# Coloquinte/sleekit

Measured on AMD Instinct MI355X. Metric: Mweights/sec quantized (GPTQ 3-bit, 4096x4096 layer), higher is better.
Workload: dtype f64

## Files before the change

### sleekit_amd/csrc/api.hip

```cpp
#include "mfma32.h"
#include "mfma64.h"

namespace slk {

__global__ __launch_bounds__(256) void k_probe_f64(double *sink, int iters) {
    double4_t c0 = {0, 0, 0, 0}, c1 = c0, c2 = c0, c3 = c0;
    const double a = 1.0 + threadIdx.x * 1e-3, b = 1.0 - threadIdx.x * 1e-3;
    for (int i = 0; i < iters; ++i) {
        c0 = __builtin_amdgcn_mfma_f64_16x16x4f64(a, b, c0, 0, 0, 0);
        c1 = __builtin_amdgcn_mfma_f64_16x16x4f64(b, a, c1, 0, 0, 0);
        c2 = __builtin_amdgcn_mfma_f64_16x16x4f64(a, a, c2, 0, 0, 0);
        c3 = __builtin_amdgcn_mfma_f64_16x16x4f64(b, b, c3, 0, 0, 0);
    }
    const double4_t s = c0 + c1 + c2 + c3;
    if (s[0] + s[1] + s[2] + s[3] == 12345.678) sink[0] = s[0];
}

template <int NACC>
__global__ __launch_bounds__(256) void k_probe_f64_n(double *sink, int iters) {
    double4_t c[NACC];
    double a[NACC], b[NACC];
#pragma unroll
    for (int i = 0; i < NACC; ++i) {
        c[i] = (double4_t){0, 0, 0, 0};
// ... 51 lines not shown
    } else if (mode == 6) {
        CHAIN(x0 = (double)(float)x0 * a;)
    } else if (mode == 7) {
        CHAIN(x0 = __longlong_as_double(((long long)__builtin_amdgcn_readlane((int)(__double_as_longlong(x0) >> 32), 5) << 32) | 7) * a;)
    } else {
        CHAIN(f = rintf(f * 1.0000001f) + 0.25f;)
    }
#undef CHAIN
    const unsigned long long t1 = __builtin_amdgcn_s_memtime(), r1 = __builtin_amdgcn_s_memrealtime();
    if (threadIdx.x == 0) {
        out[0] = (double)(t1 - t0);
        out[1] = (double)(r1 - r0);
        out[2] = x0 + x1 + x2 + x3 + x4 + x5 + x6 + x7 + f;
    }
}

}

using namespace slk;

extern "C" {

int slk_probe_chain(double *out, int iters, int mode, slk_stream_t stream) {
    SLK_REQUIRE(out && iters > 0, "bad arguments");
    hipStream_t s = as_stream(stream);
    SLK_RUN("probe_chain", 0, 0, s, k_probe_chain<<<1, 64, 0, s>>>(out, iters, mode));
    return SLK_OK;
}

size_t slk_workspace_bytes(int R, int n) {
    if (R < 0 || n <= 0) return 0;
    const size_t ld = (size_t)slk_factor_ld(n);
    const size_t rn = (size_t)(R > 0 ? R : 1) * (size_t)n;
    size_t factor = 2 * ld * ld * sizeof(double) + 2 * (ld / 64) * sizeof(int);
    size_t loop = 2 * rn * sizeof(float) + (size_t)n * sizeof(int) + 64 * sizeof(float) + 5 * 256;
    size_t search = rn * sizeof(float) + (size_t)(R + n) * sizeof(float) + (size_t)R * ((n + 127) / 128) * sizeof(float) + 4096;
    size_t error = 6 * (rn + 128 * (size_t)n) + 6 * (size_t)n * n + 4 * (size_t)R * ((n + 127) / 128) * sizeof(float) + 8192;
    size_t prep = 64 * sizeof(float) + (size_t)n * (sizeof(double) + 1);
    search += error;
    size_t m = factor;
    if (loop > m) m = loop;
    if (search > m) m = search;
    if (error > m) m = error;
    if (prep > m) m = prep;
    return m + (1u << 16);
}

size_t slk_workspace_bytes_batch(int batch, int rows_per_layer, int n) {
    if (batch < 1 || batch > 64 || rows_per_layer < 0 || n <= 0 || (long long)batch * rows_per_layer > 0x7fffffffLL) return 0;
    return slk_workspace_bytes(batch * rows_per_layer, n) + (size_t)(batch - 1) * 6 * (size_t)n * n +
           (size_t)batch * n * (sizeof(int) + sizeof(float)) + (size_t)(batch - 1) * 64 * sizeof(float) +
           4096;
}

int slk_probe_mfma_f64(double *sink, int blocks, int iters, slk_stream_t stream) {
    SLK_REQUIRE(sink && blocks > 0 && iters > 0, "bad arguments");
    hipStream_t s = as_stream(stream);
    SLK_RUN("probe_mfma_f64", 4.0 * 2048 * 4 * iters * blocks, 0, s, k_probe_f64<<<blocks, 256, 0, s>>>(sink, iters));
    return SLK_OK;
}

int slk_probe_mfma_f64_acc(double *sink, int blocks, int iters, int nacc, slk_stream_t stream) {
    SLK_REQUIRE(sink && blocks > 0 && iters > 0 && (nacc == 1 || nacc == 2 || nacc == 4 || nacc == 8 || nacc == 16), "bad arguments");
    hipStream_t s = as_stream(stream);
    if (nacc == 1)
        SLK_RUN("probe_mfma_f64", 1.0 * 2048 * 4 * iters * blocks, 0, s, k_probe_f64_n<1><<<blocks, 256, 0, s>>>(sink, iters));
    else if (nacc == 2)
        SLK_RUN("probe_mfma_f64", 2.0 * 2048 * 4 * iters * blocks, 0, s, k_probe_f64_n<2><<<blocks, 256, 0, s>>>(sink, iters));
    else if (nacc == 4)
        SLK_RUN("probe_mfma_f64", 4.0 * 2048 * 4 * iters * blocks, 0, s, k_probe_f64_n<4><<<blocks, 256, 0, s>>>(sink, iters));
    else if (nacc == 8)
        SLK_RUN("probe_mfma_f64", 8.0 * 2048 * 4 * iters * blocks, 0, s, k_probe_f64_n<8><<<blocks, 256, 0, s>>>(sink, iters));
    else
        SLK_RUN("probe_mfma_f64", 16.0 * 2048 * 4 * iters * blocks, 0, s, k_probe_f64_n<16><<<blocks, 256, 0, s>>>(sink, iters));
    return SLK_OK;
}

int slk_probe_mfma_f32(float *sink, int blocks, int iters, slk_stream_t stream) {
    SLK_REQUIRE(sink && blocks > 0 && iters > 0, "bad arguments");
    hipStream_t s = as_stream(stream);
    SLK_RUN("probe_mfma_f32", 4.0 * 4096 * 4 * iters * blocks, 0, s, k_probe_f32<<<blocks, 256, 0, s>>>(sink, iters));
    return SLK_OK;
}

}

#include <atomic>
#include <map>
#include <mutex>
#include <string>
#include <vector>
#include <strings.h>

namespace slk {
namespace {
const char *const kOptNames[OPT_COUNT] = {
    "NO_FAST_LEAF", "NO_DEFER", "NO_WINDOW2", "WIN_DBG", "NO_REGULAR_SEARCH", "NO_FAST_SEARCH_DIV",
    "NO_ERROR_SPLITK", "ERROR_CB", "NO_SYM_ERROR", "NO_BF16_ERROR", "NO_BF16_DMA", "NO_BF16_HESSIAN",
    "ERROR_F32_BELOW", "NO_BF16_ASYM", "NO_SYM_AVERAGE", "NO_WAVE_SEARCH", "LOOKAHEAD", "WINDOW_ROWS", "PANEL_SPLIT", "ROWS_BELOW_WIDE",
    "NO_LOOP_ERROR", "CHAIN_CARRIES_BELOW",
};
std::atomic<int> g_opts[OPT_COUNT];
std::once_flag g_opts_once;
void opts_from_env() {
    for (int i = 0; i < OPT_COUNT; ++i) {
        const std::string name = std::string("SLK_") + kOptNames[i];
        const char *v = getenv(name.c_str());
        int val = 0;
        if (v) {
            val = atoi(v);
            if (val == 0 && v[0] != '0') val = 1;
        }
        g_opts[i].store(val, std::memory_order_relaxed);
    }
}
int opt_index(const char *name) {
    if (!name) return -1;
    if (strncasecmp(name, "SLK_", 4) == 0) name += 4;
    for (int i = 0; i < OPT_COUNT; ++i)
        if (strcasecmp(name, kOptNames[i]) == 0) return i;
    return -1;
}
std::mutex g_lds_mu;
std::map<std::pair<const void *, int>, size_t> g_lds_set;
}

int opt(Opt o) {
    std::call_once(g_opts_once, opts_from_env);
    return g_opts[o].load(std::memory_order_relaxed);
}

namespace {
std::mutex g_helper_mu;
// ... 206 lines not shown
```

### sleekit_amd/csrc/common.h

```cpp
#pragma once

#include <hip/hip_runtime.h>
#include <stddef.h>
#include <stdint.h>
#include <stdio.h>

#include <type_traits>

#include "../../include/sleekit_amd.h"

namespace slk {

void set_error(const char *fmt, ...);

#define SLK_REQUIRE(cond, ...)          \
    do {                                \
        if (!(cond)) {                  \
            slk::set_error(__VA_ARGS__); \
            return SLK_E_ARG;           \
        }                               \
    } while (0)

#define SLK_HIP(call)                                                                  \
    do {                                                                               \
// ... 23 lines not shown
        }                                                        \
        SLK_LAUNCH_CHECK();                                      \
    } while (0)

#define SLK_RUN_W(name, flops, bytes, wgs, stream, ...) \
    do {                                                \
        slk::prof_next_width((long)(wgs));              \
        SLK_RUN(name, flops, bytes, stream, __VA_ARGS__); \
    } while (0)

enum Opt {
    OPT_NO_FAST_LEAF,
    OPT_NO_DEFER,
    OPT_NO_WINDOW2,
    OPT_WIN_DBG,
    OPT_NO_REGULAR_SEARCH,
    OPT_NO_FAST_SEARCH_DIV,
    OPT_NO_ERROR_SPLITK,
    OPT_ERROR_CB,
    OPT_NO_SYM_ERROR,
    OPT_NO_BF16_ERROR,
    OPT_NO_BF16_DMA,
    OPT_NO_BF16_HESSIAN,
    OPT_ERROR_F32_BELOW,
    OPT_NO_BF16_ASYM,
    OPT_NO_SYM_AVERAGE,
    OPT_NO_WAVE_SEARCH,
    OPT_LOOKAHEAD,
    OPT_WINDOW_ROWS,
    OPT_PANEL_SPLIT,
    OPT_ROWS_BELOW_WIDE,
    OPT_NO_LOOP_ERROR,
    OPT_CHAIN_CARRIES_BELOW,
    OPT_COUNT
};
int opt(Opt o);

struct Helper {
    hipStream_t stream;
    hipStream_t stream2;
    hipEvent_t *events;
};
constexpr int HELPER_EVENTS = 512;
hipError_t helper_for(hipStream_t main, int need, Helper *out);

hipError_t lds_opt_in(const void *kernel, size_t bytes);
#define SLK_LDS_OPT_IN(kernel, bytes) SLK_HIP(slk::lds_opt_in(reinterpret_cast<const void *>(kernel), (bytes)))

struct PtrTable {
    const float *p[64];
};

constexpr int LOOP_LAYERS = 16;
struct LayerTable {
    const float *W[LOOP_LAYERS], *scale[LOOP_LAYERS];
    const long long *order[LOOP_LAYERS];
    const double *U[LOOP_LAYERS];
};
template <class T>
__device__ __forceinline__ const T *layer_base(const T *const (&column)[LOOP_LAYERS], int b, size_t stride) {
    return column[b % LOOP_LAYERS] + (size_t)(b - b % LOOP_LAYERS) * stride;
}

int row_errors_products(const float *W, const float *Q, const float *const *Hs, int batch, int rpl, int n, const int *sym_known,
                        float *row_err, float *G, void *workspace, size_t ws_bytes, slk_stream_t stream);

// ... 182 lines not shown
```

### sleekit_amd/csrc/factor.hip

```cpp
#include <stdlib.h>

#include "mfma64.h"

namespace slk {

constexpr int PANEL = 64;
constexpr int OUTER_SMALL = 256, OUTER_LARGE = 512;
constexpr int LOOKAHEAD_MIN_TILES = 24;

__device__ long long g_panel_cycles[16];

constexpr int TP = 66;

struct PanelSmem {
    double t[PANEL][TP];
    double x[PANEL][TP];
    double a21[PANEL][TP];
    double lb[PANEL][TP];
    double rdiag[PANEL];
    int early_count;
};

#ifndef NEWTON_STEPS
#define NEWTON_STEPS 2
#endif
__device__ __forceinline__ double rsqrt_newton(double d) {
    double y = __builtin_amdgcn_rsq(d);
#pragma unroll
    for (int it = 0; it < NEWTON_STEPS; ++it) {
        const double e = __builtin_fma(-(d * y), y, 1.0);
        y = __builtin_fma(0.5 * y, e, y);
    }
    return y;
}

__device__ __forceinline__ double4_t blk_load_d(const double *blk, int lane) {
    double4_t c;
#pragma unroll
    for (int r = 0; r < 4; ++r) c[r] = blk[((lane >> 4) + 4 * r) * TP + (lane & 15)];
    return c;
}
__device__ __forceinline__ void blk_store_d(double *blk, int lane, double4_t c) {
#pragma unroll
    for (int r = 0; r < 4; ++r) blk[((lane >> 4) + 4 * r) * TP + (lane & 15)] = c[r];
}
__device__ __forceinline__ double4_t blk_mma_abt(const double *a, const double *bt, double4_t acc, double sign, int lane) {
    const int o = (lane & 15) * TP + (lane >> 4);
#pragma unroll
    for (int g = 0; g < 4; ++g) acc = __builtin_amdgcn_mfma_f64_16x16x4f64(sign * a[o + 4 * g], bt[o + 4 * g], acc, 0, 0, 0);
    return acc;
}
__device__ __forceinline__ double4_t blk_mma_ab(const double *a, const double *b, double4_t acc, int lane) {
    const int oa = (lane & 15) * TP + (lane >> 4), ob = (lane >> 4) * TP + (lane & 15);
// ... 336 lines not shown
            for (int cb = 0; cb < 4; ++cb) {
                double4_t acc = {0.0, 0.0, 0.0, 0.0};
#pragma unroll
                for (int kq = 0; kq < 4; ++kq) acc = blk_mma_abt(&sm.lb[16 * wave][16 * kq], &sm.lk[16 * cb][16 * kq], acc, 1.0, lane);
                double *cp = &sm.a21[16 * wave][16 * cb];
                double4_t o = blk_load_d(cp, lane);
#pragma unroll
                for (int r = 0; r < 4; ++r) o[r] = o[r] - acc[r];
                blk_store_d(cp, lane, o);
            }
            asm volatile("s_waitcnt lgkmcnt(0)" ::: "memory");
        }
#pragma unroll
        for (int cb = 0; cb < 4; ++cb) {
            double4_t acc = {0.0, 0.0, 0.0, 0.0};
#pragma unroll
            for (int k = 0; k < 4; ++k)
                if (k <= cb) acc = blk_mma_abt(&sm.a21[16 * wave][16 * k], &sm.x[16 * cb][16 * k], acc, 1.0, lane);
#pragma unroll
            for (int r = 0; r < 4; ++r) A[(size_t)(r0 + 16 * wave + (lane >> 4) + 4 * r) * ld + k0 + 16 * cb + (lane & 15)] = acc[r];
        }
        if (rt + 1 < last) __syncthreads();
    }
}


constexpr int INFO_HANDOFF_TIMEOUT = 0x7fffffff;
constexpr bool slk_chain_addressable(int ld) { return (size_t)ld * (size_t)ld * sizeof(double) <= 0xffffffffull; }

typedef unsigned int u32x4_t __attribute__((ext_vector_type(4)));
typedef unsigned int u32x2_t __attribute__((ext_vector_type(2)));
constexpr int AUX_SC1 = 16;
constexpr int CHAIN_CARRY_CAP = 80;
constexpr bool CHAIN_CARRY_BY_RULE = true;

struct GBuf {
    __amdgpu_buffer_rsrc_t rs;
    __device__ __forceinline__ GBuf(const double *base, size_t bytes)
        : rs(__builtin_amdgcn_make_buffer_rsrc(const_cast<double *>(base), 0, (int)(bytes > 0xffffffffull ? 0xffffffffull : bytes), 0x00020000)) {}
    template <int AUX>
    __device__ __forceinline__ double2_t load2(unsigned elem) const {
        const u32x4_t v = __builtin_amdgcn_raw_buffer_load_b128(rs, elem * 8u, 0, AUX);
        return (double2_t){__hiloint2double((int)v[1], (int)v[0]), __hiloint2double((int)v[3], (int)v[2])};
    }
    template <int AUX>
    __device__ __forceinline__ void store2(unsigned elem, double2_t x) const {
        const u32x4_t v = {(unsigned)__double2loint(x[0]), (unsigned)__double2hiint(x[0]), (unsigned)__double2loint(x[1]), (unsigned)__double2hiint(x[1])};
        __builtin_amdgcn_raw_buffer_store_b128(v, rs, elem * 8u, 0, AUX);
    }
};

__device__ __forceinline__ int flag_peek(const int *p) { return __hip_atomic_load(p, __ATOMIC_RELAXED, __HIP_MEMORY_SCOPE_AGENT); }
__device__ __forceinline__ bool flag_wait(const int *p, int want) {
    bool ok = flag_peek(p) >= want;
    if (!ok) {
        const unsigned long long t0 = __builtin_amdgcn_s_memrealtime();
        for (;;) {
            __builtin_amdgcn_s_sleep(1);
            if (flag_peek(p) >= want) {
                ok = true;
                break;
            }
            if (__builtin_amdgcn_s_memrealtime() - t0 > 200000000ull) break;
        }
    }
    __builtin_amdgcn_fence(__ATOMIC_ACQUIRE, "wavefront");
    return ok;
}
__device__ __forceinline__ void flag_publish(int *p, int value) {
    asm volatile("s_waitcnt vmcnt(0)" ::: "memory");
    __syncthreads();
    if (threadIdx.x == 0) __hip_atomic_store(p, value, __ATOMIC_RELAXED, __HIP_MEMORY_SCOPE_AGENT);
}

struct TileRegs {
    double2_t v[8];
};
template <int AUX, int J0 = 0, int J1 = 8>
__device__ __forceinline__ void tile_fetch(TileRegs &r, const GBuf &g, unsigned elem0, int ld) {
    const int t = threadIdx.x;
#pragma unroll
    for (int j = J0; j < J1; ++j) r.v[j] = g.load2<AUX>(elem0 + (unsigned)(8 * j + (t >> 5)) * (unsigned)ld + 2u * (t & 31));
}
template <int J0 = 0, int J1 = 8>
__device__ __forceinline__ void tile_stash(double (*img)[TP], const TileRegs &r) {
    const int t = threadIdx.x;
#pragma unroll
    for (int j = J0; j < J1; ++j) *reinterpret_cast<double2_t *>(&img[8 * j + (t >> 5)][2 * (t & 31)]) = r.v[j];
}
template <int AUX, int J0 = 0, int J1 = 8>
__device__ __forceinline__ void tile_store_from_lds(const GBuf &g, unsigned elem0, int ld, const double (*img)[TP]) {
    const int t = threadIdx.x;
#pragma unroll
    for (int j = J0; j < J1; ++j)
        g.store2<AUX>(elem0 + (unsigned)(8 * j + (t >> 5)) * (unsigned)ld + 2u * (t & 31), *reinterpret_cast<const double2_t *>(&img[8 * j + (t >> 5)][2 * (t & 31)]));
}

template <class Early>
__device__ __forceinline__ int diag_tile_factor(PanelSmem &sm, int lane, int wave, Early rows_0_and_1_are_in) {
    auto diag_inverse = [&](int kb) {
        const int c0 = 16 * kb, c = lane & 15;
        double xv[16];
#pragma unroll
        for (int i = 0; i < 16; ++i) {
            double s = 0.0;
#pragma unroll
            for (int u = 0; u < i; ++u) s = __builtin_fma(sm.t[c0 + i][c0 + u], xv[u], s);
            xv[i] = ((c == i ? 1.0 : 0.0) - s) * sm.rdiag[c0 + i];
        }
        if (lane < 16) {
#pragma unroll
            for (int i = 0; i < 16; ++i) sm.x[c0 + i][c0 + c] = xv[i];
        }
    };
    auto block_owner = [](int rb, int cb) { return cb == 1 ? rb : (rb == 3 && cb == 2 ? 2 : 1); };
    auto block_update = [&](int rb, int cb, int kb) {
        double *c = &sm.t[16 * rb][16 * cb];
        blk_store_d(c, lane, blk_mma_abt(&sm.t[16 * rb][16 * kb], &sm.t[16 * cb][16 * kb], blk_load_d(c, lane), -1.0, lane));
    };
    auto x_inner = [&](int rb, int cb) {
        double4_t sacc = {0.0, 0.0, 0.0, 0.0};
#pragma unroll
        for (int k = 0; k < 4; ++k)
            if (k >= cb && k < rb) sacc = blk_mma_ab(&sm.t[16 * rb][16 * k], &sm.x[16 * k][16 * cb], sacc, lane);
        return sacc;
// ... 37 lines not shown
            own_writes();
            if (kb == 2) x_block(1, 0);
            if (kb == 3) {
                x_block(2, 1);
                x_block(2, 0);
            }
        } else {
#pragma unroll
            for (int rb = kb + 1; rb < 4; ++rb)
#pragma unroll
                for (int cb = kb + 1; cb <= rb; ++cb)
                    if (block_owner(rb, cb) == wave) block_update(rb, cb, kb - 1);
            if (kb == 3) rows_0_and_1_are_in(wave - 1);
        }
        __syncthreads();
        if (kb < 3) {
#pragma unroll
            for (int rb = kb + 1; rb < 4; ++rb)
                if (block_owner(rb, kb + 1) == wave) block_update(rb, kb + 1, kb);
            __syncthreads();
        }
    }
    double4_t row3 = {0.0, 0.0, 0.0, 0.0};
    if (wave == 3) diag_inverse(3);
    else row3 = x_inner(3, wave);
    __syncthreads();
    if (wave < 3) x_finish(3, wave, row3);
    __syncthreads();
    return first_bad;
}

enum ChainForm { CHAIN_ROWS, BELOW_ROWS, CHAIN_AND_BELOW };
template <int FORM>
__device__ __forceinline__ void chol_chain_walk(PanelSmem &sm, double *__restrict__ Aall, int ld, int K0, int nb, double *__restrict__ Xall,
                                                int *__restrict__ info, int *__restrict__ flags_all, int dbg) {
    const bool BELOW = FORM == BELOW_ROWS || (FORM == CHAIN_AND_BELOW && (int)blockIdx.x >= nb);
    constexpr bool WAITS = FORM != BELOW_ROWS;
    const int t = threadIdx.x, lane = t & 63, wave = t >> 6;
    const int r = FORM == BELOW_ROWS ? nb + (int)blockIdx.x : (int)blockIdx.x, nt = ld / PANEL, p0 = K0 / PANEL;
    const int rq = BELOW ? nb : r;
    const size_t mat = (size_t)ld * ld;
    double *A = Aall + (size_t)blockIdx.z * mat;
    const GBuf ga(A, mat * sizeof(double)), gx(Xall + (size_t)blockIdx.z * mat, mat * sizeof(double));
    info += blockIdx.z;
    int *xready = flags_all + (size_t)blockIdx.z * 2 * nt, *rowdone = xready + nt;
    const int row0 = K0 + PANEL * r;
    auto elem = [&](int tr, int tc) { return (unsigned)(K0 + PANEL * tr) * (unsigned)ld + (unsigned)(K0 + PANEL * tc); };
    bool alive = true;
    if (t == 0) sm.early_count = 0;
    const bool timing = !BELOW && dbg && r > 0 && blockIdx.z == 0 && wave == 0;
    long long tmark = 0;
    auto lap = [&](int slot) {
        if (timing) {
            const long long now = (long long)__builtin_readcyclecounter();
            if (lane == 0 && slot >= 0) atomicAdd(reinterpret_cast<unsigned long long *>(&g_panel_cycles[slot]), (unsigned long long)(now - tmark));
            tmark = now;
        }
    };

    double4_t tp[3];
    if (!BELOW) {
        int i = 0;
#pragma unroll
        for (int rb = 0; rb < 4; ++rb)
#pragma unroll
            for (int cb = 0; cb <= rb; ++cb, ++i)
                if ((i & 3) == wave) {
#pragma unroll
                    for (int j = 0; j < 4; ++j) {
                        const int rr = 16 * rb + (lane >> 4) + 4 * j, cc = 16 * cb + (lane & 15);
                        tp[i >> 2][j] = (r > 0 || cc <= rr) ? A[(size_t)(row0 + rr) * ld + row0 + cc] : 0.0;
                    }
                }
    }
    auto update_cn = [&](double4_t(&cn)[4]) {
#pragma unroll
        for (int cb = 0; cb < 4; ++cb) {
            double4_t acc = {0.0, 0.0, 0.0, 0.0};
#pragma unroll
            for (int kq = 0; kq < 4; ++kq) acc = blk_mma_abt(&sm.lb[16 * wave][16 * kq], &sm.t[16 * cb][16 * kq], acc, 1.0, lane);
#pragma unroll
            for (int j = 0; j < 4; ++j) cn[cb][j] = cn[cb][j] - acc[j];
        }
    };

    auto row_done = [&](int count) {
        if (BELOW) {
            asm volatile("s_waitcnt vmcnt(0)" ::: "memory");
            __syncthreads();
        } else {
            flag_publish(&rowdone[p0 + r], count);
        }
    };
    if (rq > 0) {
        TileRegs ra, rb_;
        double4_t cn[4];
        tile_fetch<0>(ra, ga, elem(r, 0), ld);
        tile_stash(sm.a21, ra);
        for (int q = 0; q < rq; ++q) {
            const bool more = q + 1 < rq;
            if (more) {
#pragma unroll
                for (int cb = 0; cb < 4; ++cb)
#pragma unroll
                    for (int j = 0; j < 4; ++j)
                        cn[cb][j] = A[(size_t)(row0 + 16 * wave + (lane >> 4) + 4 * j) * ld + K0 + PANEL * (q + 1) + 16 * cb + (lane & 15)];
                if (q > 0) {
                    if (WAITS) alive = alive && flag_wait(&rowdone[p0 + q + 1], 1);
                    tile_fetch<AUX_SC1>(ra, ga, elem(r, 0), ld);
                    tile_fetch<AUX_SC1>(rb_, ga, elem(q + 1, 0), ld);
                }
                for (int s = 0; s < q; ++s) {
                    __syncthreads();
                    tile_stash(sm.lb, ra);
                    tile_stash(sm.t, rb_);
                    __syncthreads();
                    if (s + 1 < q) {
                        if (WAITS && alive) alive = flag_wait(&rowdone[p0 + q + 1], s + 2);
                        tile_fetch<AUX_SC1>(ra, ga, elem(r, s + 1), ld);
                        tile_fetch<AUX_SC1>(rb_, ga, elem(q + 1, s + 1), ld);
                    }
                    update_cn(cn);
                }
            }
            const bool last = !BELOW && q + 1 == r;
            auto l_block = [&](int cb) {
                double4_t acc = {0.0, 0.0, 0.0, 0.0};
#pragma unroll
                for (int k = 0; k < 4; ++k)
                    if (k <= cb) acc = blk_mma_abt(&sm.a21[16 * wave][16 * k], &sm.x[16 * cb][16 * k], acc, 1.0, lane);
                blk_store_d(&sm.lb[16 * wave][16 * cb], lane, acc);
            };
            double4_t tacc[3];
            auto t_terms = [&](int kq0, int kq1) {
                int i = 0;
#pragma unroll
                for (int rb = 0; rb < 4; ++rb)
#pragma unroll
                    for (int cb = 0; cb <= rb; ++cb, ++i)
                        if ((i & 3) == wave) {
                            double4_t acc = kq0 == 0 ? (double4_t){0.0, 0.0, 0.0, 0.0} : tacc[i >> 2];
#pragma unroll
                            for (int kq = 0; kq < 4; ++kq)
                                if (kq >= kq0 && kq < kq1) acc = blk_mma_abt(&sm.lb[16 * rb][16 * kq], &sm.lb[16 * cb][16 * kq], acc, 1.0, lane);
                            tacc[i >> 2] = acc;
                        }
            };
            if (WAITS && alive) alive = flag_wait(&xready[p0 + q], 1);
            tile_fetch<AUX_SC1, 0, 4>(ra, gx, elem(q, q), ld);
            __syncthreads();
            tile_stash<0, 4>(sm.x, ra);
            __syncthreads();
            l_block(0);
            l_block(1);
            __syncthreads();
            if (!BELOW) t_terms(0, 2);
            if (WAITS && alive) alive = flag_wait(&xready[p0 + q], 2);
            if (last) lap(-1);
            tile_fetch<AUX_SC1, 4, 8>(ra, gx, elem(q, q), ld);
            tile_stash<4, 8>(sm.x, ra);
            __syncthreads();
            if (last) lap(0);
            l_block(2);
            l_block(3);
            __syncthreads();
            if (last) lap(1);
            tile_store_from_lds<AUX_SC1>(ga, elem(r, q), ld, sm.lb);
            if (!BELOW) {
                t_terms(2, 4);
                int i = 0;
#pragma unroll
                for (int rb = 0; rb < 4; ++rb)
#pragma unroll
                    for (int cb = 0; cb <= rb; ++cb, ++i)
                        if ((i & 3) == wave) {
#pragma unroll
                            for (int j = 0; j < 4; ++j) tp[i >> 2][j] = tp[i >> 2][j] - tacc[i >> 2][j];
                            if (last) blk_store_d(&sm.t[16 * rb][16 * cb], lane, tp[i >> 2]);
                        }
            }
            if (more) {
                if (WAITS && alive) alive = flag_wait(&rowdone[p0 + q + 1], q + 1);
                tile_fetch<AUX_SC1>(rb_, ga, elem(q + 1, q), ld);
                tile_stash(sm.t, rb_);
                row_done(q + 1);
                update_cn(cn);
#pragma unroll
                for (int cb = 0; cb < 4; ++cb) blk_store_d(&sm.a21[16 * wave][16 * cb], lane, cn[cb]);
            } else {
                lap(2);
                row_done(q + 1);
                lap(3);
            }
        }
    } else if (!BELOW) {
        int i = 0;
#pragma unroll
        for (int rb = 0; rb < 4; ++rb)
#pragma unroll
            for (int cb = 0; cb <= rb; ++cb, ++i)
                if ((i & 3) == wave) blk_store_d(&sm.t[16 * rb][16 * cb], lane, tp[i >> 2]);
        for (int e = t; e < PANEL * PANEL; e += 256) sm.x[e >> 6][e & 63] = 0.0;
        __syncthreads();
    }
    if (BELOW) {
        if (WAITS && !alive && t == 0) __hip_atomic_store(info, INFO_HANDOFF_TIMEOUT, __ATOMIC_RELAXED, __HIP_MEMORY_SCOPE_AGENT);
        return;
    }
    lap(4);
    const int first_bad = diag_tile_factor(sm, lane, wave, [&](int rowblock) {
#pragma unroll
        for (int j = 0; j < 8; ++j) {
            const int row = 16 * rowblock + 2 * j + (lane >> 5);
            gx.store2<AUX_SC1>(elem(r, r) + (unsigned)row * (unsigned)ld + 2u * (lane & 31), *reinterpret_cast<const double2_t *>(&sm.x[row][2 * (lane & 31)]));
        }
        asm volatile("s_waitcnt vmcnt(0)" ::: "memory");
        int arrived = 0;
        if (lane == 0) arrived = __hip_atomic_fetch_add(&sm.early_count, 1, __ATOMIC_RELAXED, __HIP_MEMORY_SCOPE_WORKGROUP);
        arrived = __builtin_amdgcn_readfirstlane(arrived);
        if (arrived == 1) {
            if (lane == 0) __hip_atomic_store(&xready[p0 + r], 1, __ATOMIC_RELAXED, __HIP_MEMORY_SCOPE_AGENT);
            asm volatile("s_waitcnt vmcnt(0)" ::: "memory");
        }
    });
    lap(5);
    if (t == 0) {
        int expect = 0;
        if (!alive) {
            __hip_atomic_store(info, INFO_HANDOFF_TIMEOUT, __ATOMIC_RELAXED, __HIP_MEMORY_SCOPE_AGENT);
        } else if (first_bad != PANEL) {
            __hip_atomic_compare_exchange_strong(info, &expect, row0 + first_bad + 1, __ATOMIC_RELAXED, __ATOMIC_RELAXED, __HIP_MEMORY_SCOPE_AGENT);
        }
    }
    tile_store_from_lds<AUX_SC1, 4, 8>(gx, elem(r, r), ld, sm.x);
    flag_publish(&xready[p0 + r], 2);
    lap(6);
    if (timing && lane == 0) atomicAdd(reinterpret_cast<unsigned long long *>(&g_panel_cycles[15]), 1ull);
}

template <bool BELOW>
__global__ __launch_bounds__(256) void k_chol_chain(double *__restrict__ Aall, int ld, int K0, int nb, double *__restrict__ Xall,
                                                    int *__restrict__ info, int *__restrict__ flags_all, int dbg) {
    extern __shared__ __attribute__((aligned(16))) char smem_raw[];
    chol_chain_walk<BELOW ? BELOW_ROWS : CHAIN_ROWS>(*reinterpret_cast<PanelSmem *>(smem_raw), Aall, ld, K0, nb, Xall, info, flags_all, dbg);
}
__global__ __launch_bounds__(256) void k_chol_chain_below(double *__restrict__ Aall, int ld, int K0, int nb, double *__restrict__ Xall,
                                                          int *__restrict__ info, int *__restrict__ flags_all, int dbg) {
    extern __shared__ __attribute__((aligned(16))) char smem_raw[];
    chol_chain_walk<CHAIN_AND_BELOW>(*reinterpret_cast<PanelSmem *>(smem_raw), Aall, ld, K0, nb, Xall, info, flags_all, dbg);
}

struct RowsBelowSmem {
    double own[8][16][TP];
    double bt[PANEL][TP];
    double c[16][TP];
};
__global__ __launch_bounds__(256) void k_chol_rows_below(double *__restrict__ Aall, int ld, int K0, int nb, const double *__restrict__ Xall) {
    extern __shared__ __attribute__((aligned(16))) char smem_raw[];
    RowsBelowSmem &sm = *reinterpret_cast<RowsBelowSmem *>(smem_raw);
    const int t = threadIdx.x, lane = t & 63, wave = t >> 6;
    const size_t mat = (size_t)ld * ld;
    double *A = Aall + (size_t)blockIdx.z * mat;
    const GBuf ga(A, mat * sizeof(double)), gx(Xall + (size_t)blockIdx.z * mat, mat * sizeof(double));
    const int rows0 = K0 + PANEL * nb + 16 * blockIdx.x;
    auto tile_elem = [&](int tr, int tc) { return (unsigned)(K0 + PANEL * tr) * (unsigned)ld + (unsigned)(K0 + PANEL * tc); };
    auto load_c = [&](int q) {
        const double *p = A + (size_t)(rows0 + (lane >> 4)) * ld + K0 + PANEL * q + 16 * wave + (lane & 15);
        return (double4_t){p[0], p[(size_t)4 * ld], p[(size_t)8 * ld], p[(size_t)12 * ld]};
    };
    TileRegs nx;
    tile_fetch<0>(nx, gx, tile_elem(0, 0), ld);
    double4_t c = load_c(0), cnext = load_c(nb > 1 ? 1 : 0);
    for (int q = 0; q < nb; ++q) {
        for (int s = 0; s <= q; ++s) {
            const bool tri = s == q;
            __syncthreads();
            tile_stash(sm.bt, nx);
            if (tri) blk_store_d(&sm.c[0][16 * wave], lane, c);
            __syncthreads();
            if (!tri) {
                if (s + 1 < q) tile_fetch<0>(nx, ga, tile_elem(q, s + 1), ld);
                else tile_fetch<0>(nx, gx, tile_elem(q, q), ld);
// ... 99 lines not shown
    }
}

__global__ __launch_bounds__(256) void k_flip_out(const double *__restrict__ X, int ld, int n,
                                                  double *__restrict__ U) {
    X += (size_t)blockIdx.z * ld * ld;
    U += (size_t)blockIdx.z * n * n;
    for (int i = blockIdx.x; i < n; i += gridDim.x) {
        const double *src = X + (size_t)(n - 1 - i) * ld;
        double *dst = U + (size_t)i * n;
        for (int j = threadIdx.x; j < n; j += blockDim.x) dst[j] = (j >= i) ? src[n - 1 - j] : 0.0;
    }
}

__global__ void k_clear_info(int *info, int *flags, int per_matrix) {
    if (threadIdx.x == 0) info[blockIdx.x] = 0;
    if (flags)
        for (int i = threadIdx.x; i < per_matrix; i += blockDim.x) flags[(size_t)blockIdx.x * per_matrix + i] = 0;
}

}

using namespace slk;

static int chol_inverse_impl(double *A, int batch, int n, double *U, int *info, void *workspace, size_t ws_bytes,
                             slk_stream_t stream, bool want_lookahead) {
    const int ld = slk_factor_ld(n);
    const int nt = ld / TILE;
    const unsigned B = (unsigned)batch;
    const double Bd = (double)batch;
    Arena ws(workspace, ws_bytes);
    double *X = ws.take<double>((size_t)ld * ld * batch);
    double *S = ws.take<double>((size_t)ld * ld * batch);
    int *flags = ws.take<int>((size_t)batch * 2 * nt);
    if (!X || !S || !flags) {
        set_error("workspace too small for %d factorisation(s) of %d x %d", batch, n, n);
        return SLK_E_WS;
    }
    hipStream_t s = as_stream(stream);
    const int OUTER = n >= 4096 ? OUTER_LARGE : OUTER_SMALL;
    SLK_LDS_OPT_IN(k_chol_panel, sizeof(PanelSmem));
    SLK_RUN_W("clear_info", 0, 4, 1, s, k_clear_info<<<B, 64, 0, s>>>(info, flags, 2 * nt));

    Helper helper{};
    const bool lookahead = (want_lookahead || opt(OPT_LOOKAHEAD)) && nt >= LOOKAHEAD_MIN_TILES + OUTER / TILE && nt / (OUTER / TILE) < HELPER_EVENTS / 3;
    if (lookahead) SLK_HIP(helper_for(s, 3 * (nt / (OUTER / TILE) + 1), &helper));
    const int sp = opt(OPT_PANEL_SPLIT);
    const bool chain = (sp == 0 || sp == 3) && slk_chain_addressable(ld);
    const bool split = !chain && !want_lookahead && sp != 2 && (sp == 1 || batch > 1 || n >= 8192);
    if (split) SLK_LDS_OPT_IN(k_panel_below, sizeof(BelowSmem));
    if (chain) {
        SLK_LDS_OPT_IN(k_chol_chain<false>, sizeof(PanelSmem));
        SLK_LDS_OPT_IN(k_chol_chain<true>, sizeof(PanelSmem));
        SLK_LDS_OPT_IN(k_chol_chain_below, sizeof(PanelSmem));
        SLK_LDS_OPT_IN(k_chol_rows_below, sizeof(RowsBelowSmem));
    }
    int inv_done[2][16] = {{0}, {0}};
    auto inverse_nodes = [&](int tiles_done, hipStream_t st) -> int {
        int li = 0;
        for (int lvl = 1; lvl < nt; lvl *= 2, ++li) {
            const int all = (nt + 2 * lvl - 1) / (2 * lvl);
            for (int stage = 0; stage < 2; ++stage) {
                int ready;
                if (tiles_done >= nt) ready = all;
                else if (stage == 0) ready = tiles_done >= lvl ? (tiles_done - lvl) / (2 * lvl) + 1 : 0;
                else ready = tiles_done / (2 * lvl);
                if (ready > all) ready = all;
                const int first = inv_done[stage][li], count = ready - first;
                if (count <= 0) continue;
                inv_done[stage][li] = ready;
                double fl = 0, tiles = 0;
                for (int nd = first; nd < ready; ++nd) {
                    const int lo = nd * 2 * lvl, mid = lo + lvl, hi = lo + 2 * lvl < nt ? lo + 2 * lvl : nt;
                    for (int bi = mid; bi < hi; ++bi)
                        for (int bj = lo; bj < mid; ++bj) {
                            fl += 2.0 * 64 * 64 * 64 * (stage == 0 ? mid - bj : bi + 1 - mid);
                            tiles += 1;
                        }
                }
                if (tiles == 0) continue;
                dim3 grid(count * lvl * lvl, 1, B);
                if (stage == 0)
                    SLK_RUN_W("trtri_stage0", Bd * fl, Bd * (fl / 64 * 8.0 / 2 + tiles * 8.0 * 64 * 64), tiles * batch, st,
                              k_trtri_level<0><<<grid, 256, 0, st>>>(A, X, S, ld, nt, lvl, first));
                else
                    SLK_RUN_W("trtri_stage1", Bd * fl, Bd * (fl / 64 * 8.0 / 2 + tiles * 8.0 * 64 * 64), tiles * batch, st,
                              k_trtri_level<1><<<grid, 256, 0, st>>>(A, X, S, ld, nt, lvl, first));
            }
        }
        return SLK_OK;
    };
    const int EV = chain ? 3 : 2;
    int block = 0, forked = -1;
    int inverse_on_helper = -1;
    for (int K0 = 0; K0 < ld; K0 += OUTER) {
        const int K1 = K0 + OUTER < ld ? K0 + OUTER : ld;
        if (chain) {
            const int nb = (K1 - K0) / PANEL;
            int below_tiles = (ld - K1) / PANEL;
            const double e = 64.0 * nb;
            const int cc = opt(OPT_CHAIN_CARRIES_BELOW);
            const bool carry = below_tiles > 0 && !lookahead && opt(OPT_ROWS_BELOW_WIDE) == 0 && (nb + below_tiles) * batch <= CHAIN_CARRY_CAP &&
                               (cc == 1 || (cc == 0 && CHAIN_CARRY_BY_RULE));
            if (carry) {
                SLK_RUN_W("chol_chain", Bd * (e * e * e / 3.0 + 64.0 * below_tiles * e * e), Bd * (12.0 * e * e + 16.0 * 64 * below_tiles * e + 4.0 * e * e),
                          (nb + below_tiles) * batch, s,
                          k_chol_chain_below<<<dim3(nb + below_tiles, 1, B), 256, sizeof(PanelSmem), s>>>(A, ld, K0, nb, X, info, flags, opt(OPT_WIN_DBG) & 8));
                below_tiles = 0;
            } else
                SLK_RUN_W("chol_chain", Bd * e * e * e / 3.0, Bd * 12.0 * e * e, nb * batch, s,
                          k_chol_chain<false><<<dim3(nb, 1, B), 256, sizeof(PanelSmem), s>>>(A, ld, K0, nb, X, info, flags, opt(OPT_WIN_DBG) & 8));
            if (below_tiles > 0 && forked >= 0) {
                SLK_HIP(hipStreamWaitEvent(s, helper.events[EV * forked + 1], 0));
                forked = -1;
            }
            const int rw = opt(OPT_ROWS_BELOW_WIDE);
            const bool wide = rw == 1 || (rw == 0 && 4 * below_tiles * batch >= 1024);
            if (below_tiles > 0 && wide)
                SLK_RUN_W("chol_rows_below", Bd * 64.0 * below_tiles * e * e, Bd * (16.0 * 64 * below_tiles * e + 4.0 * e * e), below_tiles * batch, s,
                          k_chol_chain<true><<<dim3(below_tiles, 1, B), 256, sizeof(PanelSmem), s>>>(A, ld, K0, nb, X, info, flags, 0));
            else if (below_tiles > 0)
                SLK_RUN_W("chol_rows_below", Bd * 64.0 * below_tiles * e * e, Bd * (16.0 * 64 * below_tiles * e + 4.0 * e * e), 4 * below_tiles * batch, s,
                          k_chol_rows_below<<<dim3(4 * below_tiles, 1, B), 256, sizeof(RowsBelowSmem), s>>>(A, ld, K0, nb, X));
        }
        for (int k0 = K0; k0 < K1 && !chain; k0 += PANEL) {
            const int below = (ld - k0) / PANEL;
            const int kprev = k0 > K0 ? k0 - PANEL : -1;
            const int rest_cols = kprev >= 0 ? (K1 - k0) / PANEL - 1 : 0;
            int rest = 0;
            for (int c = 0; c < rest_cols; ++c) rest += nt - (k0 / TILE + 1 + c);
            const double prologue = kprev >= 0 ? (double)below * 2.0 * 64 * 64 * 64 + (double)below * 2.0 * 64 * 64 * 64 : 0.0;
            if (split) {
                const double pro1 = kprev >= 0 ? 2.0 * 64 * 64 * 64 : 0.0;
                SLK_RUN_W("chol_panel", Bd * (2.0 / 3.0 * 64 * 64 * 64 + pro1), Bd * 16.0 * 64 * 64, batch, s,
                          k_chol_panel<<<dim3(1, 1, B), 256, sizeof(PanelSmem), s>>>(A, ld, k0, kprev, 1, 0, X, info, opt(OPT_WIN_DBG) & 8));
                if (below - 1 + rest > 0) {
                    const int per_wg = 2;
                    const int nbw = (below - 1 + per_wg - 1) / per_wg;
                    SLK_RUN_W("chol_panel_below",
                              Bd * ((double)(below - 1) * 64 * 64 * 64 + (kprev >= 0 ? (double)(below - 1) * 2.0 * 64 * 64 * 64 : 0.0) +
                                    (double)rest * 2.0 * 64 * 64 * PANEL),
                              Bd * (24.0 * (below - 1) * 64 * 64 + (double)rest * 16.0 * 64 * 64), (nbw + rest) * batch, s,
                              k_panel_below<<<dim3(nbw + rest, 1, B), 256, sizeof(BelowSmem), s>>>(A, ld, k0, kprev, nbw, rest_cols, X, below - 1,
                                                                                                  per_wg));
// ... 81 lines not shown
                                      size_t ws_bytes, slk_stream_t stream) {
    SLK_REQUIRE(A && U && info && n > 0, "bad arguments");
    return chol_inverse_impl(A, 1, n, U, info, workspace, ws_bytes, stream, false);
}

extern "C" int slk_chol_inverse_upper_lookahead(double *A, int n, double *U, int *info, void *workspace,
                                                size_t ws_bytes, slk_stream_t stream) {
    SLK_REQUIRE(A && U && info && n > 0, "bad arguments");
    return chol_inverse_impl(A, 1, n, U, info, workspace, ws_bytes, stream, true);
}

extern "C" int slk_chol_inverse_upper_batch(double *A, int batch, int n, double *U, int *info, void *workspace,
                                            size_t ws_bytes, slk_stream_t stream) {
    SLK_REQUIRE(A && U && info && n > 0, "bad arguments");
    SLK_REQUIRE(batch >= 1 && batch <= 64, "batch must be 1..64");
    return chol_inverse_impl(A, batch, n, U, info, workspace, ws_bytes, stream, false);
}

extern "C" int slk_probe_panel_cycles(long long *host_out, int reset) {
    SLK_REQUIRE(host_out, "null pointer");
    SLK_HIP(hipDeviceSynchronize());
    SLK_HIP(hipMemcpyFromSymbol(host_out, HIP_SYMBOL(g_panel_cycles), sizeof(long long) * 16));
    if (reset) {
        long long zero[16] = {0};
        SLK_HIP(hipMemcpyToSymbol(HIP_SYMBOL(g_panel_cycles), zero, sizeof(zero)));
    }
    return SLK_OK;
}

extern "C" size_t slk_factor_workspace_bytes_batch(int batch, int n) {
    if (batch < 1 || batch > 64 || n <= 0) return 0;
    const size_t ld = (size_t)slk_factor_ld(n);
    return 2 * ld * ld * sizeof(double) * batch + (size_t)batch * (64 * sizeof(float) + (size_t)n * (sizeof(double) + sizeof(int))) +
           (size_t)batch * 2 * (ld / 64) * sizeof(int) + (1u << 16);
}
```

Measured before the change: 6536.

## Assign chain roles via atomic ticket so blocks can walk multiple rows

Chain Cholesky kernels now take their row roles from a per-panel atomic ticket counter instead of using blockIdx, which allows an optional grid smaller than the number of roles in which each block loops over several rows in ticket order. With default settings (CHAIN_GRID=0) the grid still equals the role count, so each block takes one ticket plus an extra atomic and barrier. The change also adds wait-cycle instrumentation and a third flag row in the workspace. The intent is to make dependency-ordered dispatch deadlock-safe and allow experiments with smaller grids, at the cost of slightly more synchronisation per block.

```diff
diff --git a/sleekit_amd/csrc/api.hip b/sleekit_amd/csrc/api.hip
--- a/sleekit_amd/csrc/api.hip
+++ b/sleekit_amd/csrc/api.hip
@@ -107,7 +107,7 @@
     if (R < 0 || n <= 0) return 0;
     const size_t ld = (size_t)slk_factor_ld(n);
     const size_t rn = (size_t)(R > 0 ? R : 1) * (size_t)n;
-    size_t factor = 2 * ld * ld * sizeof(double) + 2 * (ld / 64) * sizeof(int);
+    size_t factor = 2 * ld * ld * sizeof(double) + 3 * (ld / 64) * sizeof(int);
     size_t loop = 2 * rn * sizeof(float) + (size_t)n * sizeof(int) + 64 * sizeof(float) + 5 * 256;
     size_t search = rn * sizeof(float) + (size_t)(R + n) * sizeof(float) + (size_t)R * ((n + 127) / 128) * sizeof(float) + 4096;
     size_t error = 6 * (rn + 128 * (size_t)n) + 6 * (size_t)n * n + 4 * (size_t)R * ((n + 127) / 128) * sizeof(float) + 8192;
@@ -173,7 +173,7 @@
     "NO_FAST_LEAF", "NO_DEFER", "NO_WINDOW2", "WIN_DBG", "NO_REGULAR_SEARCH", "NO_FAST_SEARCH_DIV",
     "NO_ERROR_SPLITK", "ERROR_CB", "NO_SYM_ERROR", "NO_BF16_ERROR", "NO_BF16_DMA", "NO_BF16_HESSIAN",
     "ERROR_F32_BELOW", "NO_BF16_ASYM", "NO_SYM_AVERAGE", "NO_WAVE_SEARCH", "LOOKAHEAD", "WINDOW_ROWS", "PANEL_SPLIT", "ROWS_BELOW_WIDE",
-    "NO_LOOP_ERROR", "CHAIN_CARRIES_BELOW",
+    "NO_LOOP_ERROR", "CHAIN_CARRIES_BELOW", "CHAIN_GRID",
 };
 std::atomic<int> g_opts[OPT_COUNT];
 std::once_flag g_opts_once;
diff --git a/sleekit_amd/csrc/common.h b/sleekit_amd/csrc/common.h
--- a/sleekit_amd/csrc/common.h
+++ b/sleekit_amd/csrc/common.h
@@ -79,6 +79,7 @@
     OPT_ROWS_BELOW_WIDE,
     OPT_NO_LOOP_ERROR,
     OPT_CHAIN_CARRIES_BELOW,
+    OPT_CHAIN_GRID,
     OPT_COUNT
 };
 int opt(Opt o);
diff --git a/sleekit_amd/csrc/factor.hip b/sleekit_amd/csrc/factor.hip
--- a/sleekit_amd/csrc/factor.hip
+++ b/sleekit_amd/csrc/factor.hip
@@ -19,6 +19,8 @@
     double lb[PANEL][TP];
     double rdiag[PANEL];
     int early_count;
+    int role;
+    int gave_up;
 };
 
 #ifndef NEWTON_STEPS
@@ -421,6 +423,7 @@
 typedef unsigned int u32x2_t __attribute__((ext_vector_type(2)));
 constexpr int AUX_SC1 = 16;
 constexpr int CHAIN_CARRY_CAP = 80;
+constexpr int CHAIN_FLAG_ROWS = 3;
 constexpr bool CHAIN_CARRY_BY_RULE = true;
 
 struct GBuf {
@@ -456,30 +459,27 @@
     __builtin_amdgcn_fence(__ATOMIC_ACQUIRE, "wavefront");
     return ok;
 }
-__device__ __forceinline__ void flag_publish(int *p, int value) {
+__device__ __forceinline__ void flag_publish(int *p, int value, int t = threadIdx.x) {
     asm volatile("s_waitcnt vmcnt(0)" ::: "memory");
     __syncthreads();
-    if (threadIdx.x == 0) __hip_atomic_store(p, value, __ATOMIC_RELAXED, __HIP_MEMORY_SCOPE_AGENT);
+    if (t == 0) __hip_atomic_store(p, value, __ATOMIC_RELAXED, __HIP_MEMORY_SCOPE_AGENT);
 }
 
 struct TileRegs {
     double2_t v[8];
 };
 template <int AUX, int J0 = 0, int J1 = 8>
-__device__ __forceinline__ void tile_fetch(TileRegs &r, const GBuf &g, unsigned elem0, int ld) {
-    const int t = threadIdx.x;
+__device__ __forceinline__ void tile_fetch(TileRegs &r, const GBuf &g, unsigned elem0, int ld, int t = threadIdx.x) {
 #pragma unroll
     for (int j = J0; j < J1; ++j) r.v[j] = g.load2<AUX>(elem0 + (unsigned)(8 * j + (t >> 5)) * (unsigned)ld + 2u * (t & 31));
 }
 template <int J0 = 0, int J1 = 8>
-__device__ __forceinline__ void tile_stash(double (*img)[TP], const TileRegs &r) {
-    const int t = threadIdx.x;
+__device__ __forceinline__ void tile_stash(double (*img)[TP], const TileRegs &r, int t = threadIdx.x) {
 #pragma unroll
     for (int j = J0; j < J1; ++j) *reinterpret_cast<double2_t *>(&img[8 * j + (t >> 5)][2 * (t & 31)]) = r.v[j];
 }
 template <int AUX, int J0 = 0, int J1 = 8>
-__device__ __forceinline__ void tile_store_from_lds(const GBuf &g, unsigned elem0, int ld, const double (*img)[TP]) {
-    const int t = threadIdx.x;
+__device__ __forceinline__ void tile_store_from_lds(const GBuf &g, unsigned elem0, int ld, const double (*img)[TP], int t = threadIdx.x) {
 #pragma unroll
     for (int j = J0; j < J1; ++j)
         g.store2<AUX>(elem0 + (unsigned)(8 * j + (t >> 5)) * (unsigned)ld + 2u * (t & 31), *reinterpret_cast<const double2_t *>(&img[8 * j + (t >> 5)][2 * (t & 31)]));
@@ -583,22 +583,25 @@
 
 enum ChainForm { CHAIN_ROWS, BELOW_ROWS, CHAIN_AND_BELOW };
 template <int FORM>
-__device__ __forceinline__ void chol_chain_walk(PanelSmem &sm, double *__restrict__ Aall, int ld, int K0, int nb, double *__restrict__ Xall,
-                                                int *__restrict__ info, int *__restrict__ flags_all, int dbg) {
-    const bool BELOW = FORM == BELOW_ROWS || (FORM == CHAIN_AND_BELOW && (int)blockIdx.x >= nb);
+__device__ __forceinline__ void chol_chain_walk(PanelSmem &sm, const int r, const int t, double *__restrict__ Aall, int ld, int K0, int nb,
+                                                double *__restrict__ Xall, int *__restrict__ info, int *__restrict__ flags_all, int dbg) {
+    const bool BELOW = FORM == BELOW_ROWS || (FORM == CHAIN_AND_BELOW && r >= nb);
     constexpr bool WAITS = FORM != BELOW_ROWS;
-    const int t = threadIdx.x, lane = t & 63, wave = t >> 6;
-    const int r = FORM == BELOW_ROWS ? nb + (int)blockIdx.x : (int)blockIdx.x, nt = ld / PANEL, p0 = K0 / PANEL;
+    const int lane = t & 63, wave = t >> 6;
+    const int nt = ld / PANEL, p0 = K0 / PANEL;
     const int rq = BELOW ? nb : r;
     const size_t mat = (size_t)ld * ld;
     double *A = Aall + (size_t)blockIdx.z * mat;
     const GBuf ga(A, mat * sizeof(double)), gx(Xall + (size_t)blockIdx.z * mat, mat * sizeof(double));
     info += blockIdx.z;
-    int *xready = flags_all + (size_t)blockIdx.z * 2 * nt, *rowdone = xready + nt;
+    int *xready = flags_all + (size_t)blockIdx.z * CHAIN_FLAG_ROWS * nt, *rowdone = xready + nt;
     const int row0 = K0 + PANEL * r;
     auto elem = [&](int tr, int tc) { return (unsigned)(K0 + PANEL * tr) * (unsigned)ld + (unsigned)(K0 + PANEL * tc); };
     bool alive = true;
-    if (t == 0) sm.early_count = 0;
+    if (t == 0) {
+        sm.early_count = 0;
+        if (WAITS) sm.gave_up = 0;
+    }
     const bool timing = !BELOW && dbg && r > 0 && blockIdx.z == 0 && wave == 0;
     long long tmark = 0;
     auto lap = [&](int slot) {
@@ -608,6 +611,21 @@
             tmark = now;
         }
     };
+    const bool wait_timing = WAITS && dbg && wave == 0;
+    long long waited = 0;
+    auto wait = [&](const int *p, int want) {
+        const long long t0 = wait_timing ? (long long)__builtin_readcyclecounter() : 0;
+        const bool ok = flag_wait(p, want);
+        if (wait_timing) waited += (long long)__builtin_readcyclecounter() - t0;
+        return ok;
+    };
+    auto role_walked = [&]() {
+        if (wait_timing && lane == 0) {
+            const int slot = FORM == CHAIN_ROWS ? 7 : (BELOW ? 10 : 9);
+            atomicAdd(reinterpret_cast<unsigned long long *>(&g_panel_cycles[slot]), (unsigned long long)waited);
+            atomicAdd(reinterpret_cast<unsigned long long *>(&g_panel_cycles[FORM == CHAIN_ROWS ? 8 : slot + 2]), 1ull);
+        }
+    };
 
     double4_t tp[3];
     if (!BELOW) {
@@ -640,14 +658,14 @@
             asm volatile("s_waitcnt vmcnt(0)" ::: "memory");
             __syncthreads();
         } else {
-            flag_publish(&rowdone[p0 + r], count);
+            flag_publish(&rowdone[p0 + r], count, t);
         }
     };
     if (rq > 0) {
         TileRegs ra, rb_;
         double4_t cn[4];
-        tile_fetch<0>(ra, ga, elem(r, 0), ld);
-        tile_stash(sm.a21, ra);
+        tile_fetch<0>(ra, ga, elem(r, 0), ld, t);
+        tile_stash(sm.a21, ra, t);
         for (int q = 0; q < rq; ++q) {
             const bool more = q + 1 < rq;
             if (more) {
@@ -657,19 +675,19 @@
                     for (int j = 0; j < 4; ++j)
                         cn[cb][j] = A[(size_t)(row0 + 16 * wave + (lane >> 4) + 4 * j) * ld + K0 + PANEL * (q + 1) + 16 * cb + (lane & 15)];
                 if (q > 0) {
-                    if (WAITS) alive = alive && flag_wait(&rowdone[p0 + q + 1], 1);
-                    tile_fetch<AUX_SC1>(ra, ga, elem(r, 0), ld);
-                    tile_fetch<AUX_SC1>(rb_, ga, elem(q + 1, 0), ld);
+                    if (WAITS) alive = alive && wait(&rowdone[p0 + q + 1], 1);
+                    tile_fetch<AUX_SC1>(ra, ga, elem(r, 0), ld, t);
+                    tile_fetch<AUX_SC1>(rb_, ga, elem(q + 1, 0), ld, t);
                 }
                 for (int s = 0; s < q; ++s) {
                     __syncthreads();
-                    tile_stash(sm.lb, ra);
-                    tile_stash(sm.t, rb_);
+                    tile_stash(sm.lb, ra, t);
+                    tile_stash(sm.t, rb_, t);
                     __syncthreads();
                     if (s + 1 < q) {
-                        if (WAITS && alive) alive = flag_wait(&rowdone[p0 + q + 1], s + 2);
-                        tile_fetch<AUX_SC1>(ra, ga, elem(r, s + 1), ld);
-                        tile_fetch<AUX_SC1>(rb_, ga, elem(q + 1, s + 1), ld);
+                        if (WAITS && alive) alive = wait(&rowdone[p0 + q + 1], s + 2);
+                        tile_fetch<AUX_SC1>(ra, ga, elem(r, s + 1), ld, t);
+                        tile_fetch<AUX_SC1>(rb_, ga, elem(q + 1, s + 1), ld, t);
                     }
                     update_cn(cn);
                 }
@@ -697,26 +715,26 @@
                             tacc[i >> 2] = acc;
                         }
             };
-            if (WAITS && alive) alive = flag_wait(&xready[p0 + q], 1);
-            tile_fetch<AUX_SC1, 0, 4>(ra, gx, elem(q, q), ld);
+            if (WAITS && alive) alive = wait(&xready[p0 + q], 1);
+            tile_fetch<AUX_SC1, 0, 4>(ra, gx, elem(q, q), ld, t);
             __syncthreads();
-            tile_stash<0, 4>(sm.x, ra);
+            tile_stash<0, 4>(sm.x, ra, t);
             __syncthreads();
             l_block(0);
             l_block(1);
             __syncthreads();
             if (!BELOW) t_terms(0, 2);
-            if (WAITS && alive) alive = flag_wait(&xready[p0 + q], 2);
+            if (WAITS && alive) alive = wait(&xready[p0 + q], 2);
             if (last) lap(-1);
-            tile_fetch<AUX_SC1, 4, 8>(ra, gx, elem(q, q), ld);
-            tile_stash<4, 8>(sm.x, ra);
+            tile_fetch<AUX_SC1, 4, 8>(ra, gx, elem(q, q), ld, t);
+            tile_stash<4, 8>(sm.x, ra, t);
             __syncthreads();
             if (last) lap(0);
             l_block(2);
             l_block(3);
             __syncthreads();
             if (last) lap(1);
-            tile_store_from_lds<AUX_SC1>(ga, elem(r, q), ld, sm.lb);
+            tile_store_from_lds<AUX_SC1>(ga, elem(r, q), ld, sm.lb, t);
             if (!BELOW) {
                 t_terms(2, 4);
                 int i = 0;
@@ -731,9 +749,9 @@
                         }
             }
             if (more) {
-                if (WAITS && alive) alive = flag_wait(&rowdone[p0 + q + 1], q + 1);
-                tile_fetch<AUX_SC1>(rb_, ga, elem(q + 1, q), ld);
-                tile_stash(sm.t, rb_);
+                if (WAITS && alive) alive = wait(&rowdone[p0 + q + 1], q + 1);
+                tile_fetch<AUX_SC1>(rb_, ga, elem(q + 1, q), ld, t);
+                tile_stash(sm.t, rb_, t);
                 row_done(q + 1);
                 update_cn(cn);
 #pragma unroll
@@ -754,8 +772,13 @@
         for (int e = t; e < PANEL * PANEL; e += 256) sm.x[e >> 6][e & 63] = 0.0;
         __syncthreads();
     }
+    if (WAITS && !alive && lane == 0) sm.gave_up = 1;
     if (BELOW) {
-        if (WAITS && !alive && t == 0) __hip_atomic_store(info, INFO_HANDOFF_TIMEOUT, __ATOMIC_RELAXED, __HIP_MEMORY_SCOPE_AGENT);
+        if (WAITS) {
+            __syncthreads();
+            if (t == 0 && sm.gave_up) __hip_atomic_store(info, INFO_HANDOFF_TIMEOUT, __ATOMIC_RELAXED, __HIP_MEMORY_SCOPE_AGENT);
+            role_walked();
+        }
         return;
     }
     lap(4);
@@ -777,28 +800,53 @@
     lap(5);
     if (t == 0) {
         int expect = 0;
-        if (!alive) {
+        if (WAITS && sm.gave_up) {
             __hip_atomic_store(info, INFO_HANDOFF_TIMEOUT, __ATOMIC_RELAXED, __HIP_MEMORY_SCOPE_AGENT);
         } else if (first_bad != PANEL) {
             __hip_atomic_compare_exchange_strong(info, &expect, row0 + first_bad + 1, __ATOMIC_RELAXED, __ATOMIC_RELAXED, __HIP_MEMORY_SCOPE_AGENT);
         }
     }
-    tile_store_from_lds<AUX_SC1, 4, 8>(gx, elem(r, r), ld, sm.x);
-    flag_publish(&xready[p0 + r], 2);
+    tile_store_from_lds<AUX_SC1, 4, 8>(gx, elem(r, r), ld, sm.x, t);
+    flag_publish(&xready[p0 + r], 2, t);
     lap(6);
     if (timing && lane == 0) atomicAdd(reinterpret_cast<unsigned long long *>(&g_panel_cycles[15]), 1ull);
+    role_walked();
+}
+
+template <int FORM>
+__device__ __forceinline__ void chol_chain_roles(PanelSmem &sm, int roles, double *__restrict__ Aall, int ld, int K0, int nb,
+                                                 double *__restrict__ Xall, int *__restrict__ info, int *__restrict__ flags_all, int dbg) {
+    int *ticket = flags_all + ((size_t)blockIdx.z * CHAIN_FLAG_ROWS + 2) * (ld / PANEL) + K0 / PANEL;
+    int walked = 0;
+    for (;;) {
+        if (threadIdx.x == 0) sm.role = __hip_atomic_fetch_add(ticket, 1, __ATOMIC_RELAXED, __HIP_MEMORY_SCOPE_AGENT);
+        __syncthreads();
+        const int r = __builtin_amdgcn_readfirstlane(sm.role);
+        if (r >= roles) break;
+        int t = threadIdx.x;
+        asm volatile("" : "+v"(t));
+        chol_chain_walk<FORM>(sm, r, t, Aall, ld, K0, nb, Xall, info, flags_all, dbg);
+        ++walked;
+        __syncthreads();
+    }
+    if (FORM == CHAIN_AND_BELOW && dbg && threadIdx.x == 0) {
+        if (walked) atomicAdd(reinterpret_cast<unsigned long long *>(&g_panel_cycles[13]), 1ull);
+        atomicAdd(reinterpret_cast<unsigned long long *>(&g_panel_cycles[14]), 1ull);
+    }
 }
 
 template <bool BELOW>
 __global__ __launch_bounds__(256) void k_chol_chain(double *__restrict__ Aall, int ld, int K0, int nb, double *__restrict__ Xall,
                                                     int *__restrict__ info, int *__restrict__ flags_all, int dbg) {
     extern __shared__ __attribute__((aligned(16))) char smem_raw[];
-    chol_chain_walk<BELOW ? BELOW_ROWS : CHAIN_ROWS>(*reinterpret_cast<PanelSmem *>(smem_raw), Aall, ld, K0, nb, Xall, info, flags_all, dbg);
-}
-__global__ __launch_bounds__(256) void k_chol_chain_below(double *__restrict__ Aall, int ld, int K0, int nb, double *__restrict__ Xall,
+    PanelSmem &sm = *reinterpret_cast<PanelSmem *>(smem_raw);
+    if constexpr (BELOW) chol_chain_walk<BELOW_ROWS>(sm, nb + (int)blockIdx.x, threadIdx.x, Aall, ld, K0, nb, Xall, info, flags_all, dbg);
+    else chol_chain_roles<CHAIN_ROWS>(sm, nb, Aall, ld, K0, nb, Xall, info, flags_all, dbg);
+}
+__global__ __launch_bounds__(256) void k_chol_chain_below(double *__restrict__ Aall, int ld, int K0, int nb, int roles, double *__restrict__ Xall,
                                                           int *__restrict__ info, int *__restrict__ flags_all, int dbg) {
     extern __shared__ __attribute__((aligned(16))) char smem_raw[];
-    chol_chain_walk<CHAIN_AND_BELOW>(*reinterpret_cast<PanelSmem *>(smem_raw), Aall, ld, K0, nb, Xall, info, flags_all, dbg);
+    chol_chain_roles<CHAIN_AND_BELOW>(*reinterpret_cast<PanelSmem *>(smem_raw), roles, Aall, ld, K0, nb, Xall, info, flags_all, dbg);
 }
 
 struct RowsBelowSmem {
@@ -964,7 +1012,7 @@
     Arena ws(workspace, ws_bytes);
     double *X = ws.take<double>((size_t)ld * ld * batch);
     double *S = ws.take<double>((size_t)ld * ld * batch);
-    int *flags = ws.take<int>((size_t)batch * 2 * nt);
+    int *flags = ws.take<int>((size_t)batch * CHAIN_FLAG_ROWS * nt);
     if (!X || !S || !flags) {
         set_error("workspace too small for %d factorisation(s) of %d x %d", batch, n, n);
         return SLK_E_WS;
@@ -972,7 +1020,7 @@
     hipStream_t s = as_stream(stream);
     const int OUTER = n >= 4096 ? OUTER_LARGE : OUTER_SMALL;
     SLK_LDS_OPT_IN(k_chol_panel, sizeof(PanelSmem));
-    SLK_RUN_W("clear_info", 0, 4, 1, s, k_clear_info<<<B, 64, 0, s>>>(info, flags, 2 * nt));
+    SLK_RUN_W("clear_info", 0, 4, 1, s, k_clear_info<<<B, 64, 0, s>>>(info, flags, CHAIN_FLAG_ROWS * nt));
 
     Helper helper{};
     const bool lookahead = (want_lookahead || opt(OPT_LOOKAHEAD)) && nt >= LOOKAHEAD_MIN_TILES + OUTER / TILE && nt / (OUTER / TILE) < HELPER_EVENTS / 3;
@@ -1034,14 +1082,17 @@
             const int cc = opt(OPT_CHAIN_CARRIES_BELOW);
             const bool carry = below_tiles > 0 && !lookahead && opt(OPT_ROWS_BELOW_WIDE) == 0 && (nb + below_tiles) * batch <= CHAIN_CARRY_CAP &&
                                (cc == 1 || (cc == 0 && CHAIN_CARRY_BY_RULE));
+            const int cg = opt(OPT_CHAIN_GRID);
+            auto grid_of = [&](int roles) { return cg > 0 && cg < roles ? cg : roles; };
             if (carry) {
+                const int roles = nb + below_tiles, grid = grid_of(roles);
                 SLK_RUN_W("chol_chain", Bd * (e * e * e / 3.0 + 64.0 * below_tiles * e * e), Bd * (12.0 * e * e + 16.0 * 64 * below_tiles * e + 4.0 * e * e),
-                          (nb + below_tiles) * batch, s,
-                          k_chol_chain_below<<<dim3(nb + below_tiles, 1, B), 256, sizeof(PanelSmem), s>>>(A, ld, K0, nb, X, info, flags, opt(OPT_WIN_DBG) & 8));
+                          grid * batch, s,
+                          k_chol_chain_below<<<dim3(grid, 1, B), 256, sizeof(PanelSmem), s>>>(A, ld, K0, nb, roles, X, info, flags, opt(OPT_WIN_DBG) & 8));
                 below_tiles = 0;
             } else
-                SLK_RUN_W("chol_chain", Bd * e * e * e / 3.0, Bd * 12.0 * e * e, nb * batch, s,
-                          k_chol_chain<false><<<dim3(nb, 1, B), 256, sizeof(PanelSmem), s>>>(A, ld, K0, nb, X, info, flags, opt(OPT_WIN_DBG) & 8));
+                SLK_RUN_W("chol_chain", Bd * e * e * e / 3.0, Bd * 12.0 * e * e, grid_of(nb) * batch, s,
+                          k_chol_chain<false><<<dim3(grid_of(nb), 1, B), 256, sizeof(PanelSmem), s>>>(A, ld, K0, nb, X, info, flags, opt(OPT_WIN_DBG) & 8));
             if (below_tiles > 0 && forked >= 0) {
                 SLK_HIP(hipStreamWaitEvent(s, helper.events[EV * forked + 1], 0));
                 forked = -1;
@@ -1189,5 +1240,5 @@
     if (batch < 1 || batch > 64 || n <= 0) return 0;
     const size_t ld = (size_t)slk_factor_ld(n);
     return 2 * ld * ld * sizeof(double) * batch + (size_t)batch * (64 * sizeof(float) + (size_t)n * (sizeof(double) + sizeof(int))) +
-           (size_t)batch * 2 * (ld / 64) * sizeof(int) + (1u << 16);
-}
+           (size_t)batch * 3 * (ld / 64) * sizeof(int) + (1u << 16);
+}
```

After: 6529. No clear change (-0.1%).
